# sksundaram-learning/linkerd

Measured on AMD Instinct MI355X. Metric: histogram samples ingested+summarized/sec (1M series) and % HBM peak, higher is better.
Workload: dtype u32; 1 GPU; C3: 1M series, 1e9 Zipf(s=1) samples per step, log-normal values; series_total=1000000, series_per_gpu=1000000, rotating_batches=3, parallelism=series-sharded x1 (weighted ranges), step=ingest (sample+plan+bin1+bin2) + snapshot(reset, dense counts + summaries)

## Files before the change

linkerd_amd/csrc/l5dh_engine.cpp:

```cpp
#include <algorithm>
#include <cerrno>
#include <cstring>
#include <mutex>
#include <new>
#include <string>
#include <vector>

#include "l5dh_ctx.hpp"

using namespace l5dh;

namespace {

constexpr size_t MAX_BATCH = ((size_t)1 << 30) - 65536;

hipEvent_t ev_get(l5dh_ctx* c) {
  if (!c->ev_pool.empty()) {
    hipEvent_t e = c->ev_pool.back();
    c->ev_pool.pop_back();
    return e;
  }
  hipEvent_t e = nullptr;
  hipEventCreate(&e);
  return e;
// ... 113 lines not shown
  Segs sv = segs_view(c);
  size_t recs = 0;
  for (int j = 0; j < c->nseg; ++j) recs += c->segs[j].n;
  uint32_t hc = c->hot_chunk;
  {
    const size_t fill = recs / (2 * (size_t)std::max(1, c->num_cu));
    hc = (uint32_t)std::min<size_t>(hc, std::max<size_t>(16384, (fill + 1023) & ~(size_t)1023));
  }
  if (int r = ensure(c, c->split_item, (recs / hc + 2 * (size_t)c->F + 2) * 8)) return r;
  Plan pl = plan(c);
  const int direct_out = final_mode && reset && out.counts && out.first == 0 && out.count == (uint32_t)c->S;
  if (encode && !(final_mode && reset && out.first == 0 && out.count == (uint32_t)c->S && !out.counts && !out.summ))
    return fail(c, -EINVAL, "internal: the sparse export is a whole-range resetting export");
  {
    KTimer kt(c, L5DH_K_SCAN);
    if (encode) HIPCHK(c, launch_enc_dirty(state(c), pl, c->stream));
    HIPCHK(c, launch_plan(sv, c->F, final_mode, c->cold_limit, hc, c->d_dirty, direct_out, encode ? 1 : 0, pl,
                          c->stream));
  }
  if (encode) {
    uint32_t words = 0;
    HIPCHK(c, hipMemcpyAsync(&words, c->d_header + 5 + 4 * ((c->F + 1023) / 1024), 4, hipMemcpyDeviceToHost,
                             c->stream));
    HIPCHK(c, hipStreamSynchronize(c->stream));
    if (int r = ensure(c, c->m_unpacked, (size_t)words * 4 + 16)) return r;
    c->m_unpacked_words = words;
    out.enc = c->m_unpacked.as<uint32_t>();
  }
  const uint32_t hot = (uint32_t)std::min<size_t>(c->F, recs / ((size_t)c->cold_limit + 1));
  const uint32_t split_items = (uint32_t)std::min<size_t>(0xFFFFFFF0u, recs / hc + 2 * (size_t)hot);
  State st = state(c);
  Tables tb = tables(c);
  if (hot) {
    KTimer kt(c, L5DH_K_HOT);
    HIPCHK(c, launch_hot_init(pl, hot, st, out, direct_out, c->stream));
  }
  bool joined = true;
  {
    KTimer kt(c, L5DH_K_ACCUM);
    const bool big_seen = __atomic_load_n(c->h_header + 5, __ATOMIC_RELAXED) != 0u;
    if (split_items && big_seen) {
      HIPCHK(c, hipEventRecord(c->ev_fork, c->stream));
      HIPCHK(c, hipStreamWaitEvent(c->side, c->ev_fork, 0));
      HIPCHK(c, launch_accum_split(sv, pl, split_items, st, tb, out, direct_out, hc, c->stream));
      HIPCHK(c, launch_accum_cold(sv, pl, DEV_COUNT, st, tb, out, final_mode, reset, c->side));
      HIPCHK(c, hipEventRecord(c->ev_join, c->side));
      joined = false;
    } else {
      if (split_items) HIPCHK(c, launch_accum_split(sv, pl, split_items, st, tb, out, direct_out, hc, c->stream));
      HIPCHK(c, launch_accum_cold(sv, pl, DEV_COUNT, st, tb, out, final_mode, reset, c->stream));
    }
    if (hot) HIPCHK(c, launch_hot_finish(pl, hot, st, tb, out, final_mode, reset, direct_out, c->stream));
    if (!joined) HIPCHK(c, hipStreamWaitEvent(c->stream, c->ev_join, 0));
  }
  c->nseg = 0;
  return 0;
}

int flush_ring(l5dh_ctx* c) {
  if (!c->ring_fill) return 0;
  const size_t n = c->ring_fill;
  c->ring_fill = 0;
  return do_ingest(c, c->ring_series.as<const uint32_t>(), c->ring_values.as<const float>(), n);
}

}

namespace {

int fold(l5dh_ctx* c) {
  Outputs none{nullptr, nullptr, 0, 0, nullptr};
  return aggregate(c, 0, 0, none);
}

int check_err(l5dh_ctx* c) {
  const uint32_t seen = __atomic_load_n(c->h_header + 4, __ATOMIC_ACQUIRE);
  if (seen != c->err_reported) {
    c->err_reported = seen;
    return fail(c, -EINVAL, "series id >= max_series in an ingest batch (those samples were dropped)");
  }
  return 0;
}

int do_ingest(l5dh_ctx* c, const uint32_t* series, const float* values, size_t n) {
  if (n == 0) return 0;
  if (n > MAX_BATCH) return fail(c, -EINVAL, "batch piece larger than 2^30 samples");
  if (c->nseg >= c->max_seg) {
    int r = fold(c);
    if (r) return r;
  }
  const uint32_t* ds = series;
  const float* dv = values;
  if (!is_device_ptr(series) || !is_device_ptr(values)) {
    int r;
    if ((r = ensure(c, c->stage_series, n * 4))) return r;
    if ((r = ensure(c, c->stage_values, n * 4))) return r;
    KTimer kt(c, L5DH_K_COPY);
    HIPCHK(c, hipMemcpyAsync(c->stage_series.p, series, n * 4, hipMemcpyDefault, c->stream));
    HIPCHK(c, hipMemcpyAsync(c->stage_values.p, values, n * 4, hipMemcpyDefault, c->stream));
    ds = c->stage_series.as<const uint32_t>();
    dv = c->stage_values.as<const float>();
  }
  const bool vec = ((uintptr_t)ds % 16 == 0) && ((uintptr_t)dv % 16 == 0);
  if (c->F == 1) {
    KTimer kt(c, L5DH_K_BIN);
    const size_t fill = n / (size_t)std::max(1, c->num_cu);
    const uint32_t chunk =
        (uint32_t)std::min<size_t>(c->hot_chunk & ~3u, std::max<size_t>(16384, (fill + 1023) & ~(size_t)1023));
    HIPCHK(c, launch_fold1(ds, dv, n, chunk, state(c), tables(c), c->d_err, vec, (c->variant & 1) != 0, c->stream));
    c->fold_last = n;
    HIPCHK(c, hipMemcpyAsync(c->h_header + 4, c->d_err, 4, hipMemcpyDeviceToHost, c->stream));
    return 0;
  }
  auto& sg = c->segs[c->nseg];
  const size_t cap32 = n + n / 2 + ((size_t)1 << 19);
  const size_t cap16 = 2 * n + n / 8 + (size_t)128 * c->F + 4096;
  const size_t dlim16 = (cap16 - (n + (size_t)16 * c->F + 1024)) & ~(size_t)7;
  {
    int r = ensure(c, sg.rec32, (cap32 + 16) * 4);
    if (!r) r = ensure(c, sg.rec16, (cap16 + 16) * 2);
    if (r) return r;
  }
  int G = (int)std::min<size_t>((size_t)c->G_max, (n + 8191) / 8192);
  if (G < 1) G = 1;
  size_t per = (n + G - 1) / G;
  per = (per + 3) & ~(size_t)3;
  G = (int)((n + per - 1) / per);
  IngestArgs a{};
  a.series = ds;
  a.values = dv;
  a.n = n;
  a.per = per;
  a.G = G;
  a.num_cu = c->num_cu;
  a.S = c->S;
  a.F = c->F;
  a.tb = tables(c);
  a.sumfix = c->d_sumfix;
  a.err = c->d_err;
  a.err_host = c->h_header_dev + 4;
  a.kest = c->d_kest;
  a.kprev = c->d_kprev;
  a.meta = sg.meta;
  a.rec32 = sg.rec32.as<uint32_t>();
  a.rec16 = sg.rec16.as<uint16_t>();
  a.cap32 = cap32;
  a.cap16 = cap16;
  a.dlim16 = dlim16;
  a.thr_min = (uint32_t)std::min<uint64_t>(std::max<uint64_t>(1, n / (8192ull * c->direct_div)), 0xFFFFFFFFull);
  const uint32_t FS = (c->F + 63) / 64;
  a.dmax = std::min<uint32_t>(c->direct_max, ((uint32_t)BIN1_BINS - 9 - FS) / 2);
  a.pct = c->region_pct;
  a.vec = vec;
  {
    KTimer kt(c, L5DH_K_SCAN);
    if (c->variant & 4) HIPCHK(c, hipMemsetAsync(c->d_kprev, 0, (size_t)2 * c->F * 4, c->stream));
    HIPCHK(c, launch_ingest(a, 0, c->stream));
  }
  {
    KTimer kt(c, L5DH_K_BIN);
    HIPCHK(c, launch_ingest(a, 1, c->stream));
  }
  {
    KTimer kt(c, L5DH_K_BIN2);
    HIPCHK(c, launch_ingest(a, 3, c->stream));
  }
  sg.n = n;
  c->nseg++;
  return 0;
}

int wait_inputs(l5dh_ctx* c) {
  HIPCHK(c, hipEventRecord(c->ev_copy, c->stream));
  HIPCHK(c, hipEventSynchronize(c->ev_copy));
  return 0;
}

int issue_ticket(l5dh_ctx* c, uint64_t* ticket) {
  const uint64_t t = ++c->tick_next;
  const int slot = (int)(t % l5dh_ctx::NTICK);
  if (!c->tick_ev[slot]) HIPCHK(c, hipEventCreateWithFlags(&c->tick_ev[slot], hipEventDisableTiming));
  HIPCHK(c, hipEventRecord(c->tick_ev[slot], c->stream));
  c->tick_of[slot] = t;
  *ticket = t;
  return 0;
}

int wait_ticket(l5dh_ctx* c, uint64_t t) {
  if (t <= c->tick_done) return 0;
  if (t > c->tick_next) return fail(c, -EINVAL, "unknown ingest ticket");
  const int slot = (int)(t % l5dh_ctx::NTICK);
  HIPCHK(c, hipEventSynchronize(c->tick_ev[slot]));
  c->tick_done = std::max(c->tick_done, c->tick_of[slot]);
  return 0;
}

int ingest_impl(l5dh_ctx* c, const uint32_t* series, const float* values, size_t n, uint64_t* ticket = nullptr) {
  if (ticket) *ticket = c->tick_next;
  if (n == 0) return 0;
  const bool dev = is_device_ptr(series) && is_device_ptr(values);
  const bool wait = (!dev || c->stream == c->own_stream) && !ticket;
  if (c->ring_cap && n <= c->ring_cap / 2) {
    int r;
    if (c->ring_fill + n > c->ring_cap && (r = flush_ring(c))) return r;
    if ((r = ensure(c, c->ring_series, c->ring_cap * 4 + 64)) || (r = ensure(c, c->ring_values, c->ring_cap * 4 + 64)))
      return r;
    {
      KTimer kt(c, L5DH_K_COPY);
      uint32_t* rs = c->ring_series.as<uint32_t>() + c->ring_fill;
      float* rv = c->ring_values.as<float>() + c->ring_fill;
      const void* hs = dev || (c->variant & 2) ? nullptr : host_mapped_ptr(series);
      const void* hv = hs ? host_mapped_ptr(values) : nullptr;
      if (hs && hv) {
        HIPCHK(c, launch_fetch_host(static_cast<const uint32_t*>(hs), static_cast<const uint32_t*>(hv), rs,
                                    reinterpret_cast<uint32_t*>(rv), n, c->stream));
      } else {
        HIPCHK(c, hipMemcpyAsync(rs, series, n * 4, hipMemcpyDefault, c->stream));
        HIPCHK(c, hipMemcpyAsync(rv, values, n * 4, hipMemcpyDefault, c->stream));
      }
    }
    c->ring_fill += n;
    if (ticket) return issue_ticket(c, ticket);
    return wait ? wait_inputs(c) : 0;
  }
  int r = flush_ring(c);
  if (r) return r;
  for (size_t o = 0; o < n; o += MAX_BATCH) {
    const size_t m = std::min(n - o, MAX_BATCH);
    if ((r = do_ingest(c, series + o, values + o, m))) return r;
  }
  if (ticket) return issue_ticket(c, ticket);
  return wait ? wait_inputs(c) : 0;
}

bool full_range(l5dh_ctx* c, uint32_t first, uint32_t count) { return first == 0 && count == c->S; }

int do_snapshot(l5dh_ctx* c, uint32_t first, uint32_t count, l5dh_summary* out, int32_t* counts_out, int reset) {
  if ((uint64_t)first + count > c->S) return fail(c, -EINVAL, "series range out of bounds");
  if (count == 0) return 0;
  int r = flush_ring(c);
  if (r) return r;
  StagedOut<Summary88> summ;
  StagedOut<int32_t> cnt;
  if ((r = summ.begin(c, out, count, c->stage_summ)) || (r = cnt.begin(c, counts_out, (size_t)count * NB, c->stage_counts)))
    return r;
  Outputs o{summ.dev, cnt.dev, first, count, nullptr};
  if (full_range(c, first, count) && c->F > 1) {
    if ((r = aggregate(c, 1, reset, o))) return r;
  } else {
    if ((r = fold(c))) return r;
    KTimer kt(c, L5DH_K_HOT);
    HIPCHK(c, launch_rows(state(c), nullptr, nullptr, tables(c), o, reset, nullptr, c->stream));
  }
  {
    KTimer kt(c, L5DH_K_COPY);
    if ((r = summ.end(c)) || (r = cnt.end(c))) return r;
  }
  if (!summ.staged() && !cnt.staged() && c->stream != c->own_stream) return 0;
  return sync_stream(c);
}

int do_rollup(l5dh_ctx* c, uint32_t first, uint32_t count, const int32_t* ext, const int64_t* ext_totals,
              const uint32_t* group, uint32_t G, l5dh_summary* g_out, int32_t* g_counts_out, int64_t* g_totals_out,
              l5dh_summary* series_out, int reset) {
  int r;
  const bool live = ext == nullptr;
  if (live && ((r = flush_ring(c)) || (r = fold(c)))) return r;
  RollupWork w{};
  w.count = count;
  w.G = G;
  w.first = first;
  w.item = c->rollup_item;
  w.caps = rollup_caps(count, G, w.item);
  w.tmp_bytes = rollup_tmp_bytes(G);
  const size_t G1 = (size_t)G + 1;
  if ((r = ensure(c, c->ru_u32, (4 * G1 + RH_WORDS) * 4)) || (r = ensure(c, c->ru_u64, 2 * G1 * 8)) ||
      (r = ensure(c, c->ru_members, ((size_t)count + 1) * 4)) || (r = ensure(c, c->ru_igroup, w.caps.items * 4)) ||
      (r = ensure(c, c->ru_mlist, (w.caps.multi + 1) * 4)) ||
      (r = ensure(c, c->ru_partial, (w.caps.slots + 1) * (size_t)RU_PROW * 8)) ||
      (r = ensure(c, c->ru_tmp, w.tmp_bytes)))
    return r;
  {
    KTimer kt(c, L5DH_K_COPY);
    if ((r = stage_in(c, group, count, 4, c->ru_group)) ||
        (r = stage_in(c, ext, (size_t)count * NB, 8, c->stage_in_counts)) ||
        (r = stage_in(c, ext_totals, count, 8, c->stage_in_totals)))
      return r;
  }
  w.group = group;
  uint32_t* u = c->ru_u32.as<uint32_t>();
  w.cnt = u;
  w.nitems = u + G1;
  w.cursor = u + 2 * G1;
  w.pbase = u + 3 * G1;
  w.hdr = u + 4 * G1;
  w.moff = c->ru_u64.as<uint64_t>();
  w.ioff = w.moff + G1;
  w.members = c->ru_members.as<uint32_t>();
  w.igroup = c->ru_igroup.as<uint32_t>();
  w.mlist = c->ru_mlist.as<uint32_t>();
  w.partial = c->ru_partial.as<uint64_t>();
  w.tmp = c->ru_tmp.p;
  StagedOut<Summary88> g_summ, s_summ;
  StagedOut<int32_t> g_cnt;
  StagedOut<int64_t> g_tot;
  if ((r = g_summ.begin(c, g_out, G, c->ru_summ)) || (r = g_cnt.begin(c, g_counts_out, (size_t)G * NB, c->ru_counts)) ||
// ... 507 lines not shown
```

linkerd_amd/csrc/l5dh_ingest.hip:

```cpp
#include <algorithm>
#include <type_traits>

#include "l5dh_device.hpp"

namespace l5dh {
namespace {

constexpr uint32_t RSAMPLE = 1u << 18;
#ifndef L5DH_RS_WG
#define L5DH_RS_WG 64
#endif
constexpr int RS_WG = L5DH_RS_WG;
static_assert((RSAMPLE + RS_WG - 1) / RS_WG <= 65535, "k_rsample's u16 LDS counters: at most 65535 draws per workgroup");
constexpr uint32_t INVALID = 0xFFFFFFFFu;

__device__ __forceinline__ uint32_t round_up(uint32_t x, uint32_t m) { return (x + m - 1) / m * m; }

__device__ __forceinline__ uint32_t rcap(double prev, double e, double s, bool exact, double pad, uint32_t align,
                                         uint32_t pct, double z, bool floor_sample) {
  double c;
  if (exact) {
    c = e;
  } else {
    const double e0 = prev / s, sg = sqrt(e0 + 1.0);
// ... 112 lines not shown
      } else if (t < F) {
        x[i].x = kw[2 * t];
        x[i].y = kw[2 * t + 1];
      }
    }
  };
  uint2 te[16];
  {
    uint4 x[16];
    load_pairs(kest, x);
#pragma unroll
    for (int i = 0; i < 16; ++i) te[i] = make_uint2(x[i].x + x[i].y, x[i].z + x[i].w);
  }
  auto scaled = [&](uint32_t v) -> uint32_t { return (uint32_t)fmin((double)v * s, 4294967295.0); };
  __syncthreads();
  RP_MARK(1)
  auto hist = [&](uint32_t v) {
    const uint32_t e = scaled(v);
    const bool ok = dmax > 0 && e >= thr_min && e > 0;
    const int bin = ok ? 31 - __clz((int)e) : 0;
    const uint64_t act = __ballot(ok);
    if (!act) return;
    const int b0 = __builtin_amdgcn_readlane(bin, __builtin_ctzll(act));
    if (__ballot(ok && bin == b0) == act) {
      if (lane == 0) atomicAdd(&lh[b0], (uint32_t)__popcll(act));
    } else if (ok) {
      atomicAdd(&lh[bin], 1u);
    }
  };
#pragma unroll
  for (int i = 0; i < 16; ++i) {
    hist(te[i].x);
    hist(te[i].y);
  }
  __syncthreads();
  if (j < 64) {
    const uint32_t c = j < 32 ? lh[31 - j] : 0u;
    const uint32_t cum = wave_incl_scan32(c);
    const uint64_t ok = __ballot(dmax > 0 && j < 32 && cum <= dmax);
    const int nb = __popcll(ok);
    if (j == 0) sthr = nb ? max(max(thr_min, 1u), 1u << (32 - nb)) : 0xFFFFFFFFu;
  }
#pragma unroll
  for (int i = 0; i < 16; ++i) reinterpret_cast<uint2*>(tw)[j + 1024u * (uint32_t)i] = te[i];
  uint4 xp[16];
  load_pairs(kprev, xp);
  __syncthreads();
  const uint32_t thr = sthr;
  RP_MARK(2)
  uint32_t dbits = 0, E = 0;
#pragma unroll
  for (int k = 0; k < 32; ++k) {
    const uint32_t kk = (uint32_t)(k + (int)j) & 31u;
    const uint32_t v = tw[t0 + kk];
    if (t0 + kk < F && scaled(v) >= thr) dbits |= 1u << kk;
    else E += v;
  }
  __syncthreads();
#pragma unroll
  for (int i = 0; i < 16; ++i)
    reinterpret_cast<uint2*>(tw)[j + 1024u * (uint32_t)i] = make_uint2(xp[i].x + xp[i].y, xp[i].z + xp[i].w);
  __syncthreads();
  uint64_t P = 0;
#pragma unroll
  for (int k = 0; k < 32; ++k) {
    const uint32_t kk = (uint32_t)(k + (int)j) & 31u;
    if (!((dbits >> kk) & 1u)) P += tw[t0 + kk];
  }
  RP_MARK(3)
  uint32_t cv[4] = {(uint32_t)__popc(dbits), 0u, 0u, 0u}, ct[4];
  block_excl_scan4<1024>(cv, lds4, ct);
  const uint32_t ND = ct[0];
  meta[L.dbits() + j] = j < NW ? dbits : 0u;
  meta[L.dpre() + j] = cv[0];
  {
    uint32_t x = dbits, di = cv[0];
    while (x) {
      const uint32_t k = (uint32_t)(__ffs((int)x) - 1);
      x &= x - 1u;
      dl[di] = t0 + k;
      meta[L.dlist() + di] = t0 + k;
      ++di;
    }
  }
  P += __shfl_xor(P, 1, 64);
  E += __shfl_xor(E, 1, 64);
  RP_MARK(4)
  if ((j & 1u) == 0 && (j >> 1) < FS) {
    const uint32_t b = j >> 1;
    capl[b] = rcap((double)P, (double)E, s, exact, 256.0, 4, pct, 6.0, true);
    meta[L.btot() + b] = (uint32_t)min(P, (uint64_t)0xFFFFFFFFu);
  }
  __syncthreads();
  RP_MARK(5)
  const uint32_t TB = FS + 2 * ND;
  if (j >= FS && j < TB) {
    const uint32_t t = dl[(j - FS) >> 1], h = (j - FS) & 1u;
    const double p = (double)kprev[2 * t + h], e = (double)kest[2 * t + h];
    capl[j] = rcap(p, e, s, exact, 256.0, 8, pct, 5.0, false);
  }
  __syncthreads();
  const bool stb = j < FS, dj = j >= FS && j < TB;
  uint64_t tot32, tot16;
  const uint64_t base32 = block_excl_scan64(stb ? (uint64_t)capl[j] : 0ull, l64, &tot32);
  const uint64_t base16 = block_excl_scan64(dj ? (uint64_t)capl[j] : 0ull, l64, &tot16);
  const uint64_t base = stb ? base32 : base16;
  const uint64_t lim = stb ? cap32 : dlim16;
  if (base + capl[j] + 16 > lim)
    capl[j] = base + 16 < lim ? (uint32_t)(lim - 16 - base) & (stb ? ~3u : ~7u) : 0u;
  meta[L.bbase() + j] = (uint32_t)base;
  meta[L.bcap() + j] = j < TB ? capl[j] : 0u;
  meta[L.bcnt() + j] = 0u;
  if (j == 0) {
    uint32_t* hdr = meta + L.hdr();
    hdr[H_ND] = ND;
    hdr[H_OV1] = 0;
    hdr[H_REDO1] = 0;
    hdr[H_OV2] = 0;
    hdr[H_REDO2] = 0;
    hdr[H_COUNT2] = 0;
    hdr[H_EXACT] = exact ? 1u : 0u;
    hdr[H_D16] = (uint32_t)min(tot16, (uint64_t)dlim16);
  }
  RP_MARK(6)
}




#ifdef L5DH_PHASES
__device__ unsigned long long g_phase1[1024 * 8];
__device__ unsigned long long g_phase3[1024 * 8];
#define PH_INIT unsigned long long ph_acc[7] = {0, 0, 0, 0, 0, 0, 0}, ph_t = wall_clock64();
#define PH_VWAIT asm volatile("s_waitcnt vmcnt(0)" ::: "memory");
#define PH_MARK(k)                                 \
  if (threadIdx.x == 0) {                          \
    const unsigned long long ph_n = wall_clock64(); \
    ph_acc[k] += ph_n - ph_t;                      \
    ph_t = ph_n;                                   \
  }
#define PH_FLUSH                                                                   \
  if (threadIdx.x == 0 && pass == 0) {                                             \
    for (int k = 0; k < 7; ++k) g_phase1[blockIdx.x * 8 + k] += ph_acc[k];          \
    g_phase1[blockIdx.x * 8 + 7] += 1;                                             \
  }
#else
#define PH_INIT
#define PH_MARK(k)
#define PH_VWAIT
#define PH_FLUSH
#endif
__device__ __forceinline__ uint4 ld_stream(const uint32_t* p) { return *reinterpret_cast<const uint4*>(p); }
constexpr int CHW = 16384;
using dsum_t = unsigned long long;
constexpr uint32_t NODEST = 0xFFFFFFFFu - (uint32_t)CHW;
constexpr int NT1 = 1024;
constexpr int DSUM_N = DIRECT_MAX * TILE;
constexpr size_t rbin1w_lds() {
  return (size_t)CHW * 4 + BIN1_BINS * 12 + CHW / 8 + CHW / 32 + 1024 * 8 + LUT2_N * 8 + DSUM_N * sizeof(dsum_t);
}

template <int NT, int CH>
__global__ __launch_bounds__(NT) void k_rbin1w(const uint32_t* __restrict__ series, const float* __restrict__ values,
                                                  size_t n, size_t per, uint32_t S, uint32_t F, Tables tb,
                                                  uint32_t* __restrict__ meta, uint32_t* __restrict__ rec32,
                                                  uint16_t* __restrict__ rec16, int64_t* __restrict__ sumfix,
                                                  uint32_t* __restrict__ err, int vec, int pass) {
  constexpr int PT = CH / NT;
  constexpr int PH = PT / 2;
  constexpr int GS = 4;
  static_assert(PH % 4 == 0 && PH % GS == 0 && GS % 4 == 0 && CH <= 32768, "halves of whole 16-B groups; 15-bit ranks");
  extern __shared__ __attribute__((aligned(16))) uint32_t smem[];
  uint32_t* stage = smem;
  uint32_t* cnt = stage + CH;
  uint32_t* offr = cnt + BIN1_BINS;
  uint32_t* rdelta = offr + BIN1_BINS;
  uint32_t* heads = rdelta + BIN1_BINS;
  uint16_t* gpre = reinterpret_cast<uint16_t*>(heads + CH / 32);
  uint2* dw = reinterpret_cast<uint2*>(gpre + CH / 64);
  uint2* lut2 = dw + 1024;
  __shared__ uint32_t wsum[NT / 64];
  dsum_t* dsum = reinterpret_cast<dsum_t*>(lut2 + LUT2_N);
  const MetaLayout L = meta_layout(F);
  uint32_t* hdr = meta + L.hdr();
  if (pass == 1 && __builtin_amdgcn_readfirstlane(hdr[H_REDO1]) == 0u) return;
  uint32_t* bcnt = meta + L.bcnt();
  const uint32_t* bbase = meta + L.bbase();
  const uint32_t* bcap = meta + L.bcap();
  const uint32_t FS = (F + ST_TILES - 1) / ST_TILES;
  const uint32_t NW = (F + 31) / 32;
  const uint32_t ND = hdr[H_ND];
  const uint32_t TB = FS + 2 * ND;
  const int lane = lane_id();
  const int wv = threadIdx.x >> 6;
  for (uint32_t w = threadIdx.x; w < NW; w += NT) dw[w] = make_uint2(meta[L.dbits() + w], meta[L.dpre() + w]);
  for (uint32_t b = threadIdx.x; b < BIN1_BINS; b += NT) cnt[b] = 0;
  for (uint32_t i = threadIdx.x; i < LUT2_N; i += NT) lut2[i] = tb.lut2[i];
  for (uint32_t i = threadIdx.x; i < ND * TILE; i += NT) dsum[i] = 0;
  __syncthreads();
  const uint32_t lo = (uint32_t)((size_t)blockIdx.x * per);
  const uint32_t hi = (uint32_t)min((size_t)lo + per, n);
  bool bad = false;
  constexpr int RB0 = (BIN1_BINS + NT - 1) / NT;
  uint32_t my_base[RB0], my_cap[RB0];
#pragma unroll
  for (int j = 0; j < RB0; ++j) {
    const uint32_t b = threadIdx.x + (uint32_t)j * NT;
    my_base[j] = b < TB ? bbase[b] : 0u;
    my_cap[j] = b < TB ? bcap[b] : 0u;
  }
  PH_INIT
  constexpr int PFG = PH / 4;
  uint4 pfs[PFG], pfv[PFG];
  auto prefetch = [&](uint32_t c) {
#pragma unroll
    for (int k = 0; k < PFG; ++k) {
      const uint32_t base = c + 4u * ((uint32_t)k * NT + threadIdx.x);
      pfs[k] = ld_stream(series + base);
      pfv[k] = ld_stream(reinterpret_cast<const uint32_t*>(values) + base);
    }
  };
  if (vec && lo + (uint32_t)CH <= hi) prefetch(lo);
  for (uint32_t c0 = lo; c0 < hi; c0 += CH) {
    for (uint32_t wd = threadIdx.x; wd < CH / 32; wd += NT) heads[wd] = 0u;
    uint32_t pk[PT];
    const bool full = vec && c0 + (uint32_t)CH <= hi;
    const uint32_t cl = c0;
    uint4 hs[PH / 4], hv[PH / 4];
    auto load_second = [&]() {
      if (full) {
#pragma unroll
        for (int k = 0; k < PH / 4; ++k) {
          const uint32_t base = cl + 4u * ((uint32_t)(PH / 4 + k) * NT + threadIdx.x);
          hs[k] = ld_stream(series + base);
          hv[k] = ld_stream(reinterpret_cast<const uint32_t*>(values) + base);
        }
      }
    };
#pragma unroll
    for (int h = 0; h < 2; ++h) {
      if (h == 1) { PH_MARK(1) }
      uint32_t sv[PH];
      float fv[PH];
      if (full) {
#pragma unroll
        for (int k = 0; k < PH / 4; ++k) {
          uint4 s4, u4;
          if (h == 0) {
            s4 = pfs[h * (PH / 4) + k];
            u4 = pfv[h * (PH / 4) + k];
          } else {
            s4 = hs[k];
            u4 = hv[k];
          }
          const float4 f4 = make_float4(__uint_as_float(u4.x), __uint_as_float(u4.y), __uint_as_float(u4.z),
                                        __uint_as_float(u4.w));
          sv[4 * k] = s4.x; sv[4 * k + 1] = s4.y; sv[4 * k + 2] = s4.z; sv[4 * k + 3] = s4.w;
          fv[4 * k] = f4.x; fv[4 * k + 1] = f4.y; fv[4 * k + 2] = f4.z; fv[4 * k + 3] = f4.w;
        }
      } else {
#pragma unroll
        for (int k = 0; k < PH; ++k) {
          const uint32_t i = c0 + 4u * ((uint32_t)(h * (PH / 4) + (k >> 2)) * NT + threadIdx.x) + (uint32_t)(k & 3);
          const bool in = i < hi;
          sv[k] = in ? series[i] : 0xFFFFFFFFu;
          fv[k] = in ? values[i] : 0.0f;
          bad |= in && sv[k] >= S;
        }
      }
      if (full) {
        PH_VWAIT
        if (h == 0) { PH_MARK(0) } else { PH_MARK(2) }
      }
#pragma unroll
      for (int g = 0; g < PH; g += GS) {
        if (h == 0 && g == GS) load_second();
        uint32_t pl[GS];
        uint32_t escm = 0;
#pragma unroll
        for (int q = 0; q < GS; ++q) {
          const float f = fv[g + q];
          const bool fast = __float_as_uint(f) < 0x49FFC000u;
          pl[q] = fast ? (uint32_t)f : 0u;
          escm |= (!fast && sv[g + q] < S) ? (1u << q) : 0u;
          if (full) bad |= sv[g + q] >= S;
        }
        if (__ballot(escm != 0u)) {
#pragma unroll 1
          for (int q = 0; q < GS; ++q) {
            if ((escm >> q) & 1u) {
              const uint32_t i = cl + 4u * ((uint32_t)(h * (PH / 4) + (g + q) / 4) * NT + threadIdx.x) + (uint32_t)(q & 3);
              const uint32_t r = payload1_slow(series[i], values[i], tb, pass == 0 ? sumfix : nullptr);
#pragma unroll
              for (int u = 0; u < GS; ++u) pl[u] = q == u ? r : pl[u];
            }
          }
        }
        uint2 dv[GS], lv[GS];
#pragma unroll
        for (int q = 0; q < GS; ++q) dv[q] = dw[(sv[g + q] >> (TILE_SHIFT + 5)) & 1023u];
#pragma unroll
        for (int q = 0; q < GS; ++q) lv[q] = lut2[lut2_index(pl[q])];
        uint32_t rc4[GS];
#pragma unroll
        for (int q = 0; q < GS; ++q) {
          const uint32_t s = sv[g + q];
          const uint32_t tw = __builtin_amdgcn_ubfe(s, TILE_SHIFT, 5);
          const bool direct = s < S && __builtin_amdgcn_ubfe(dv[q].x, tw, 1) != 0u;
          const uint32_t di = dv[q].y + (uint32_t)__popc(__builtin_amdgcn_ubfe(dv[q].x, 0, tw));
          const uint32_t p = pl[q];
          uint32_t o;
          const uint32_t bk = lut2_decode(p, lv[q], o);
          const bool esc = p >= V_ESC;
          const uint32_t bucket = sel_u32(esc, p - V_ESC, bk);
          rc4[q] = sel_u32(direct, ((s & (TILE - 1)) << 11) | bucket, ((s & (ST_TILES * TILE - 1)) << 21) | p);
          const uint32_t dbin = FS + 2u * di + ((s >> 4) & 1u);
          const uint32_t bn = sel_u32(s < S, sel_u32(direct, dbin, s >> ST_SHIFT), TB);
          pk[h * PH + g + q] = atomicAdd(cnt + bn, 1u) | (bn << 15);
          if (direct && !esc && pass == 0 && p) atomicAdd(&dsum[di * TILE + (s & (TILE - 1))], (dsum_t)p);
        }
#pragma unroll
        for (int j = 0; j < GS / 4; ++j)
          *reinterpret_cast<uint4*>(stage + 4u * ((uint32_t)(h * (PH / 4) + g / 4 + j) * NT + threadIdx.x)) =
              make_uint4(rc4[4 * j], rc4[4 * j + 1], rc4[4 * j + 2], rc4[4 * j + 3]);
        asm volatile("" ::: "memory");
      }
    }
    __syncthreads();
    PH_MARK(3)
    constexpr int RB = (BIN1_BINS + NT - 1) / NT;
    uint32_t rn[RB], rold[RB], rbase[RB], rcapv[RB];
#pragma unroll
    for (int j = 0; j < RB; ++j) {
      const uint32_t rb_bin = threadIdx.x + (uint32_t)j * NT;
      rn[j] = rb_bin <= TB ? cnt[rb_bin] : 0u;
      rold[j] = 0;
      rbase[j] = my_base[j];
      rcapv[j] = my_cap[j];
      if (rb_bin < TB && rn[j]) rold[j] = atomicAdd(&bcnt[rb_bin], rn[j]);
    }
    {
      static_assert(NT == BIN1_BINS && RB == 1, "one bin per thread");
      const uint32_t pv = rn[0] | ((rn[0] ? 1u : 0u) << 16);
      const uint32_t wi = wave_incl_scan32(pv);
      if (lane == 63) wsum[wv] = wi;
      __syncthreads();
      uint32_t pre = 0;
      for (int q = 0; q < wv; ++q) pre += wsum[q];
      const uint32_t ex = pre + wi - pv;
      offr[threadIdx.x] = ex;
      if (rn[0]) atomicOr(&heads[(ex & 0xFFFFu) >> 5], 1u << (ex & 31u));
    }
    uint32_t rec[PT];
#pragma unroll
    for (int kk = 0; kk < PT / 4; ++kk) {
      const uint4 v = *reinterpret_cast<const uint4*>(stage + 4u * ((uint32_t)kk * NT + threadIdx.x));
      rec[4 * kk] = v.x; rec[4 * kk + 1] = v.y; rec[4 * kk + 2] = v.z; rec[4 * kk + 3] = v.w;
    }
    __syncthreads();
    PH_MARK(4)
    if (vec && c0 + 2u * (uint32_t)CH <= hi) prefetch(c0 + (uint32_t)CH);
#pragma unroll
    for (int k = 0; k < PT; ++k) {
      const uint32_t bin = (pk[k] >> 15) & 1023u;
      stage[(offr[bin] & 0xFFFFu) + (pk[k] & 0x7FFFu)] = rec[k];
    }
    if (wv == 0) {
      constexpr int GPL = CH / 64 / 64;
      static_assert(GPL % 2 == 0, "two groups per 16-B read");
      uint32_t pc[GPL], t = 0;
#pragma unroll
      for (int k = 0; k < GPL; k += 2) {
        const uint4 w = *reinterpret_cast<const uint4*>(heads + 2u * (GPL * (uint32_t)lane + (uint32_t)k));
        pc[k] = (uint32_t)(__popc(w.x) + __popc(w.y));
        pc[k + 1] = (uint32_t)(__popc(w.z) + __popc(w.w));
        t += pc[k] + pc[k + 1];
      }
      uint32_t ex = wave_incl_scan32(t) - t;
#pragma unroll
      for (int k = 0; k < GPL; ++k) {
        gpre[GPL * (uint32_t)lane + (uint32_t)k] = (uint16_t)ex;
        ex += pc[k];
      }
    }
#pragma unroll
    for (int j = 0; j < RB; ++j) {
      const uint32_t rb_bin = threadIdx.x + (uint32_t)j * NT;
      if (rn[j]) {
        uint32_t d = NODEST;
        if (rb_bin < TB) {
          if (rold[j] + rn[j] <= rcapv[j]) d = rbase[j] + rold[j] - (offr[rb_bin] & 0xFFFFu);
          else hdr[H_OV1] = 1u;
        }
        rdelta[offr[rb_bin] >> 16] = d;
      }
    }
    __syncthreads();
    PH_MARK(5)
    const uint32_t nst = offr[FS] >> 16;
#pragma unroll
    for (int j = 0; j < RB; ++j)
      if (threadIdx.x + (uint32_t)j * NT < BIN1_BINS) cnt[threadIdx.x + (uint32_t)j * NT] = 0;
#pragma unroll 4
    for (int k = 0; k < PT; ++k) {
      const uint32_t i = (uint32_t)wv * (PT * 64) + (uint32_t)k * 64 + (uint32_t)lane;
      const uint32_t g = i >> 6;
      const unsigned long long hw = *reinterpret_cast<const unsigned long long*>(heads + 2 * g);
      const uint32_t run = (uint32_t)gpre[g] + mask_below(hw) + (uint32_t)((hw >> lane) & 1ull) - 1u;
      const uint32_t d = rdelta[run];
      if (d != NODEST) {
        if (run < nst)
          rec32[i + d] = stage[i];
        else
          rec16[i + d] = (uint16_t)stage[i];
      }
    }
    __syncthreads();
    PH_MARK(6)
  }
  PH_FLUSH
  if (pass == 0) {
    const uint32_t* dl = meta + L.dlist();
    for (uint32_t i = threadIdx.x; i < ND * TILE; i += NT) {
      const unsigned long long v = dsum[i];
      const uint32_t s = dl[i / TILE] * TILE + (i & (TILE - 1));
      if (v && s < S) atomicAdd(reinterpret_cast<unsigned long long*>(&sumfix[s]), (unsigned long long)v);
    }
    if (bad) atomicAdd(err, 1u);
  }
}

__device__ __forceinline__ uint32_t lut3_byte(uint32_t v) {
  const uint32_t sh = 25u - (uint32_t)__builtin_clz(v | 64u);
  return ((v >> sh) + (sh << 6)) << 3;
}
__device__ __forceinline__ uint32_t lut3_bucket(uint32_t v, uint2 x) {
  return (x.x & 0x7FFu) + (((v << 11) | 0x7FFu) >= x.x ? 1u : 0u) + (v >= x.y ? 1u : 0u);
}

__global__ __launch_bounds__(1024) void k_rfix1(uint32_t F, uint32_t* __restrict__ meta, const uint32_t* __restrict__ err,
                                                uint32_t* __restrict__ err_host) {
  __shared__ uint32_t lds[17];
  const MetaLayout L = meta_layout(F);
  uint32_t* hdr = meta + L.hdr();
  if (threadIdx.x == 0) *reinterpret_cast<volatile uint32_t*>(err_host) = *err;
  const uint32_t FS = (F + ST_TILES - 1) / ST_TILES;
  const uint32_t ND = hdr[H_ND];
  const uint32_t TB = FS + 2 * ND;
  const uint32_t ov = hdr[H_OV1];
  const uint32_t b = threadIdx.x;
  const bool stb = b < FS, dj = b >= FS && b < TB;
  const uint32_t c = b < TB ? meta[L.bcnt() + b] : 0u;
  if (stb && !hdr[H_EXACT]) {
    const double P = (double)meta[L.btot() + b];
    if ((double)c > P * 1.0625 + 4.0 * sqrt(P) + 256.0) hdr[H_COUNT2] = 1u;
  }
  meta[L.btot() + b] = c;
  uint32_t t32, t16;
  const uint32_t nb32 = block_excl_scan<1024>(stb ? round_up(c, 4) : 0u, lds, &t32);
  const uint32_t nb16 = block_excl_scan<1024>(dj ? round_up(c, 8) : 0u, lds, &t16);
  const uint32_t nb = stb ? nb32 : nb16;
  const uint32_t base = ov ? nb : meta[L.bbase() + b];
  if (dj) {
    const uint32_t t = meta[L.dlist() + ((b - FS) >> 1)], h = (b - FS) & 1u;
    meta[L.kbase() + 2 * t + h] = base;
    meta[L.kcnt() + 2 * t + h] = c;
  }
  if (ov) {
    meta[L.bbase() + b] = nb;
    meta[L.bcap() + b] = round_up(c, stb ? 4 : 8);
    meta[L.bcnt() + b] = 0u;
  }
  const uint32_t d16 = hdr[H_D16];
  if (ov && t16 > d16) {
    for (uint32_t k = b; k < L.K; k += 1024)
      if (!((meta[L.dbits() + (k >> 6)] >> ((k >> 1) & 31u)) & 1u)) meta[L.kcap() + k] = 0u;
  }
  uint32_t all;
  const uint32_t is = block_excl_scan<1024>(stb ? (c + ITEM2 - 1) / ITEM2 : 0u, lds, &all);
  if (stb) meta[L.istart() + b] = is;
  __syncthreads();
  if (b == 0) {
    meta[L.istart() + FS] = all;
    hdr[H_ITEMS] = all;
    if (ov && t16 > d16) {
      hdr[H_D16] = t16;
      hdr[H_COUNT2] = 1u;
    }
    hdr[H_OV2] = 0u;
    hdr[H_REDO2] = 0u;
    hdr[H_REDO1] = ov;
    hdr[H_OV1] = 0u;
    if (ov) hdr[H_NOVR1] += 1u;
  }
}

__device__ __forceinline__ bool tile_direct(const uint32_t* __restrict__ meta, const MetaLayout& L, uint32_t t) {
  return (meta[L.dbits() + (t >> 5)] >> (t & 31u)) & 1u;
// ... 301 lines not shown
    if (wv < 2) {
      uint32_t rb = INVALID;
      if (rc) {
        if (rold + rc <= rcapv) rb = rbase + rold;
        else hdr[H_OV2] = 1u;
      }
      ocx[b * B2_KEYS + rk].y = rb;
      cnt[rk] = 0u;
    }
    __syncthreads();
    PH2_MARK(4)
    prev_total = ctot;
#pragma unroll
    for (int g = 0; g < PG; ++g) x[g] = xn[g];
  }
  write_out((int)((i1 - 1) & 1u), prev_total);
  __syncthreads();
  if (pass == 0) flush(cur_j);
#ifdef L5DH_PHASES
  if (threadIdx.x == 0 && pass == 0) {
    for (int k = 0; k < 5; ++k) g_phase3[blockIdx.x * 8 + k] += ph2[k];
    g_phase3[blockIdx.x * 8 + 7] += 1;
  }
#endif
}

__global__ __launch_bounds__(1024) void k_rfix2a(uint32_t F, uint32_t* __restrict__ meta, uint32_t* __restrict__ kprev) {
  __shared__ uint64_t red[16];
  const MetaLayout L = meta_layout(F);
  uint32_t* hdr = meta + L.hdr();
  const uint32_t k = blockIdx.x * 1024u + threadIdx.x;
  uint32_t r8 = 0;
  if (k < L.K) {
    const uint32_t c = meta[L.kcnt() + k];
    kprev[k] = c;
    if (!tile_direct(meta, L, k >> 1)) r8 = round_up(c, 8);
  }
  const uint64_t w = wave_sum((uint64_t)r8);
  if ((threadIdx.x & 63) == 0) red[threadIdx.x >> 6] = w;
  __syncthreads();
  if (threadIdx.x == 0) {
    uint64_t t = 0;
    for (int q = 0; q < 16; ++q) t += red[q];
    reinterpret_cast<uint64_t*>(meta + L.wsum())[blockIdx.x] = t;
    if (blockIdx.x == 0) hdr[H_REDO2] = hdr[H_OV2] | hdr[H_COUNT2];
  }
}

__global__ __launch_bounds__(1024) void k_rfix2b(uint32_t F, uint32_t* __restrict__ meta) {
  __shared__ uint64_t red[16];
  __shared__ uint64_t l64[17];
  const MetaLayout L = meta_layout(F);
  uint32_t* hdr = meta + L.hdr();
  if (hdr[H_REDO2] == 0u) return;
  const uint64_t before = wsum_before(reinterpret_cast<const uint64_t*>(meta + L.wsum()), blockIdx.x, red);
  const uint32_t k = blockIdx.x * 1024u + threadIdx.x;
  const bool mine = k < L.K && !tile_direct(meta, L, k >> 1);
  const uint32_t c8 = mine ? round_up(meta[L.kcnt() + k], 8) : 0u;
  uint64_t total;
  const uint64_t base = hdr[H_D16] + before + block_excl_scan64((uint64_t)c8, l64, &total);
  if (mine) {
    meta[L.kbase() + k] = (uint32_t)base;
    meta[L.kcap() + k] = c8;
    meta[L.kcnt() + k] = 0u;
  }
  if (blockIdx.x == 0 && threadIdx.x == 0) {
    if (hdr[H_COUNT2]) hdr[H_NCNT2] += 1u;
    else hdr[H_NOVR2] += 1u;
    hdr[H_OV2] = 0u;
  }
}

__global__ __launch_bounds__(1024) void k_rfix2s(uint32_t F, uint32_t* __restrict__ meta, uint32_t* __restrict__ kprev) {
  __shared__ uint64_t l64[17];
  const MetaLayout L = meta_layout(F);
  uint32_t* hdr = meta + L.hdr();
  constexpr uint32_t KPM = RFIX2_ONE_WG_MAX / 1024;
  const uint32_t KP = (L.K + 1023) / 1024, k0 = threadIdx.x * KP;
  const uint32_t redo = hdr[H_OV2] | hdr[H_COUNT2];
  const uint32_t counted = hdr[H_COUNT2];
  uint32_t c8[KPM], dm = 0;
  uint64_t mine = 0;
#pragma unroll
  for (uint32_t q = 0; q < KPM; ++q) {
    const uint32_t k = k0 + q;
    c8[q] = 0;
    if (q < KP && k < L.K) {
      const uint32_t c = meta[L.kcnt() + k];
      kprev[k] = c;
      if (tile_direct(meta, L, k >> 1)) {
        dm |= 1u << q;
      } else {
        c8[q] = round_up(c, 8);
        mine += c8[q];
      }
    }
  }
  __syncthreads();
  if (threadIdx.x == 0) hdr[H_REDO2] = redo;
  if (!redo) return;
  uint64_t total;
  uint64_t kb = (uint64_t)hdr[H_D16] + block_excl_scan64(mine, l64, &total);
#pragma unroll
  for (uint32_t q = 0; q < KPM; ++q) {
    const uint32_t k = k0 + q;
    if (q < KP && k < L.K && !((dm >> q) & 1u)) {
      meta[L.kbase() + k] = (uint32_t)kb;
      meta[L.kcap() + k] = c8[q];
      meta[L.kcnt() + k] = 0u;
      kb += c8[q];
    }
  }
  if (threadIdx.x == 0) {
    if (counted) hdr[H_NCNT2] += 1u;
    else hdr[H_NOVR2] += 1u;
    hdr[H_OV2] = 0u;
  }
}

__global__ __launch_bounds__(256) void k_fetch_host(const uint32_t* __restrict__ hs, const uint32_t* __restrict__ hv,
                                                    uint32_t* __restrict__ ds, uint32_t* __restrict__ dv, size_t n) {
  const size_t stride = (size_t)gridDim.x * blockDim.x;
  for (size_t i = (size_t)blockIdx.x * blockDim.x + threadIdx.x; i < n; i += stride) {
    const uint32_t s = hs[i], v = hv[i];
    ds[i] = s;
    dv[i] = v;
  }
}

}

#ifdef L5DH_PHASES
extern "C" __attribute__((visibility("default"))) int l5dh_dev_phases3(unsigned long long* out) {
  return (int)hipMemcpyFromSymbol(out, HIP_SYMBOL(g_phase3), sizeof(g_phase3), 0, hipMemcpyDeviceToHost);
}
extern "C" __attribute__((visibility("default"))) int l5dh_dev_phases_plan(unsigned long long* out) {
  return (int)hipMemcpyFromSymbol(out, HIP_SYMBOL(g_phase_plan), sizeof(g_phase_plan), 0, hipMemcpyDeviceToHost);
}
extern "C" __attribute__((visibility("default"))) int l5dh_dev_phases1(unsigned long long* out) {
  return (int)hipMemcpyFromSymbol(out, HIP_SYMBOL(g_phase1), sizeof(g_phase1), 0, hipMemcpyDeviceToHost);
}
#endif

hipError_t launch_fetch_host(const uint32_t* hs, const uint32_t* hv, uint32_t* ds, uint32_t* dv, size_t n,
                             hipStream_t st) {
  if (n == 0) return hipSuccess;
  const size_t blocks = std::min<size_t>((n + 255) / 256, 2048);
  hipLaunchKernelGGL(k_fetch_host, dim3((unsigned)blocks), dim3(256), 0, st, hs, hv, ds, dv, n);
  return hipGetLastError();
}

hipError_t set_ingest_attributes() {
  hipError_t e;
  if ((e = hipFuncSetAttribute((const void*)k_rsample, hipFuncAttributeMaxDynamicSharedMemorySize, 32768 * 4)))
    return e;
  if ((e = hipFuncSetAttribute((const void*)k_rplan1, hipFuncAttributeMaxDynamicSharedMemorySize, (int)RPLAN1_LDS)))
    return e;
  return hipFuncSetAttribute((const void*)k_rbin1w<NT1, CHW>, hipFuncAttributeMaxDynamicSharedMemorySize,
                             (int)rbin1w_lds());
}

hipError_t launch_ingest(const IngestArgs& a, int stage, hipStream_t st) {
  const uint32_t K = 2 * a.F;
  switch (stage) {
    case 0:
      hipLaunchKernelGGL(k_rsample, dim3(RS_WG), dim3(1024), (size_t)((K + 1) / 2) * 4, st, a.series, a.n, a.S, K,
                         a.kest);
      hipLaunchKernelGGL(k_rplan1, dim3(1), dim3(1024), RPLAN1_LDS, st, a.n, a.F, a.kest, a.kprev, a.meta, a.cap32,
                         a.dlim16, a.thr_min, a.dmax, a.pct);
      {
        const uint32_t B = (K + 1023) / 1024;
        hipLaunchKernelGGL(k_rplan2a, dim3(B), dim3(1024), 0, st, a.n, a.F, a.kest, a.kprev, a.meta, a.pct);
        hipLaunchKernelGGL(k_rplan2b, dim3(B), dim3(1024), 0, st, a.F, a.meta, a.cap16);
      }
      break;
    case 1:
      for (int pass = 0; pass < 2; ++pass) {
        hipLaunchKernelGGL((k_rbin1w<NT1, CHW>), dim3(a.G), dim3(NT1), rbin1w_lds(), st, a.series, a.values, a.n,
                           a.per, a.S, a.F, a.tb, a.meta, a.rec32, a.rec16, a.sumfix, a.err, a.vec ? 1 : 0, pass);
        if (pass == 0) hipLaunchKernelGGL(k_rfix1, dim3(1), dim3(1024), 0, st, a.F, a.meta, a.err, a.err_host);
      }
      break;
    case 2:
      break;
    default: {
      const uint32_t B = (K + 1023) / 1024;
      for (int pass = 0; pass < 2; ++pass) {
        const MetaLayout L = meta_layout(a.F);
        hipLaunchKernelGGL(k_rbin2<B2_NT>, dim3(a.num_cu * B2_PER_CU), dim3(B2_NT), 0, st, a.S, a.F, a.tb, a.meta,
                           a.meta + L.istart(), a.meta + L.bbase(), a.meta + L.btot(), a.rec32, a.rec16, a.sumfix,
                           pass);
        if (pass == 0 && K <= RFIX2_ONE_WG_MAX) {
          hipLaunchKernelGGL(k_rfix2s, dim3(1), dim3(1024), 0, st, a.F, a.meta, a.kprev);
        } else if (pass == 0) {
          hipLaunchKernelGGL(k_rfix2a, dim3(B), dim3(1024), 0, st, a.F, a.meta, a.kprev);
          hipLaunchKernelGGL(k_rfix2b, dim3(B), dim3(1024), 0, st, a.F, a.meta);
        }
      }
      break;
    }
  }
  return hipGetLastError();
}

}
```

linkerd_amd/csrc/l5dh_kernels.hpp:

```cpp
#pragma once

#include <hip/hip_runtime.h>

#include <cstddef>
#include <cstdint>

#include "l5dh_tables.hpp"

namespace l5dh {

constexpr int TILE = 32;
constexpr int TILE_SHIFT = 5;
constexpr int ST_TILES = 64;
constexpr int ST_SHIFT = 11;
constexpr int CROW = 900;
constexpr int HROW = 1800;
constexpr int MAX_SEG = 8;
constexpr int WG = 1024;
constexpr uint32_t COLD_LIMIT_MAX = 65535u;

constexpr size_t ACC_COLDH_LDS = (size_t)16 * CROW * 4 + 16 * 8 + ROW * 4;
constexpr int ENC_LIST = 256;
constexpr size_t ACC_COLDHE_LDS = ACC_COLDH_LDS + 2 * 16 * 4 + (size_t)16 * ENC_LIST * 2;
constexpr size_t ACC_SPLIT_LDS = (size_t)16 * HROW * 4;
constexpr size_t FOLD16_LDS = (size_t)16 * HROW * 4 + 16 * 64 * 8 + 1024 * 8;
constexpr size_t FOLD32_LDS = (size_t)TILE * CROW * 4 + TILE * 64 * 8 + 1024 * 8;

struct Tables {
  const int32_t* lim_pad;
  const int32_t* mid;
  const int32_t* base;
  const uint32_t* lut;
  const uint2* lut2;
  const uint2* lut3;
};

constexpr int DIRECT_MAX = 255;
constexpr int BIN1_BINS = 1024;
constexpr uint32_t ITEM2 = 6144;
struct MetaLayout {
  uint32_t K;
  __host__ __device__ constexpr uint32_t kbase() const { return 0; }
  __host__ __device__ constexpr uint32_t kcnt() const { return K; }
  __host__ __device__ constexpr uint32_t kcap() const { return 2 * K; }
  __host__ __device__ constexpr uint32_t dbits() const { return 3 * K; }
  __host__ __device__ constexpr uint32_t dpre() const { return 3 * K + 1024; }
  __host__ __device__ constexpr uint32_t dlist() const { return 3 * K + 2048; }
  __host__ __device__ constexpr uint32_t bbase() const { return 3 * K + 2304; }
  __host__ __device__ constexpr uint32_t bcnt() const { return 3 * K + 3328; }
  __host__ __device__ constexpr uint32_t bcap() const { return 3 * K + 4352; }
  __host__ __device__ constexpr uint32_t btot() const { return 3 * K + 5376; }
  __host__ __device__ constexpr uint32_t hdr() const { return 3 * K + 6400; }
  __host__ __device__ constexpr uint32_t istart() const { return 3 * K + 6464; }
  __host__ __device__ constexpr uint32_t wsum() const { return 3 * K + 6980; }
  __host__ __device__ constexpr uint32_t words() const { return 3 * K + 7108; }
};
__host__ __device__ constexpr MetaLayout meta_layout(uint32_t F) { return MetaLayout{2 * F}; }
enum : uint32_t {
  H_ND = 0,
  H_OV1 = 1,
  H_REDO1 = 2,
  H_OV2 = 3,
  H_REDO2 = 4,
  H_ITEMS = 5,
  H_COUNT2 = 6,
  H_EXACT = 9,
  H_NOVR1 = 10,
  H_NOVR2 = 11,
  H_D16 = 12,
  H_NCNT2 = 13
};
constexpr uint32_t NOKEY = 0xFFFFFFFFu;

struct Segs {
  const uint16_t* rec16[MAX_SEG];
  const uint32_t* meta[MAX_SEG];
  int n;
};

struct Summary88 {
  int64_t count, min, max, sum, p50, p90, p95, p99, p9990, p9999;
  double avg;
};
static_assert(sizeof(Summary88) == 88, "HistogramSummary layout");

struct State {
  uint32_t* counts;
  int64_t* total;
  int64_t* sumfix;
  uint8_t* dirty;
  uint32_t S, F;
};

constexpr uint32_t CI_DIRTY = 1u << 30;
constexpr uint8_t TF_SPLIT = 2;
constexpr uint8_t TF_DIRTY = 4;
constexpr uint8_t TF_SOLO = 8;

struct Plan {
  uint32_t* tile_tot;
  uint32_t* enc_base;
  uint32_t* enc_h0;
  uint32_t* enc_dw;
  uint4* cold_item;
  uint2* split_item;
  uint32_t* hot_list;
  uint8_t* tile_flags;
  uint32_t* header;
  uint32_t* big_hint;
};
__host__ __device__ constexpr uint32_t plan_header_words(uint32_t F) { return 6 + 4 * ((F + 1023) / 1024); }
constexpr uint32_t ENC_HALF_CAP = 16u * 2u * NB + 16u;
static_assert((uint64_t)((1u << 20) / TILE) * 2u * ENC_HALF_CAP < (1ull << 32),
              "the unpacked encoding's u32 word offsets (L5DH_MAX_SERIES = 2^20 series)");

struct Outputs {
  Summary88* summ;
  int32_t* counts;
  uint32_t first, count;
  int64_t* totals;
  uint32_t* words;
  uint32_t* enc;
  uint32_t* roff;
};
constexpr uint32_t MERGE_CMAX = 0x1FFFFFu;

struct IngestArgs {
  const uint32_t* series;
  const float* values;
  size_t n, per;
  int G;
  int num_cu;
  uint32_t S, F;
  Tables tb;
  int64_t* sumfix;
  uint32_t* err;
  uint32_t* err_host;
  uint32_t* kest;
  uint32_t* kprev;
  uint32_t* meta;
  uint32_t* rec32;
  uint16_t* rec16;
  size_t cap32, cap16;
  size_t dlim16;
  uint32_t thr_min, dmax;
  uint32_t pct;
  bool vec;
};
hipError_t launch_ingest(const IngestArgs& a, int stage, hipStream_t st);
hipError_t set_ingest_attributes();

hipError_t launch_fold1(const uint32_t* series, const float* values, size_t n, uint32_t chunk, State state, Tables tb,
                        uint32_t* err, bool vec, bool wide, hipStream_t st);

hipError_t launch_enc_dirty(State st, Plan plan, hipStream_t st_);
hipError_t launch_plan(Segs segs, uint32_t F, int final_mode, uint32_t cold_limit, uint32_t hot_chunk,
                       const uint8_t* dirty, int direct_out, int encode, Plan plan, hipStream_t st);
constexpr uint32_t DEV_COUNT = 0xFFFFFFFFu;
hipError_t launch_hot_init(Plan plan, uint32_t max_hot, State state, Outputs out, int direct_out, hipStream_t st);
hipError_t launch_accum_cold(Segs segs, Plan plan, uint32_t cold_items, State state, Tables tb, Outputs out,
                             int final_mode, int reset, hipStream_t st);
hipError_t launch_accum_split(Segs segs, Plan plan, uint32_t max_split_items, State state, Tables tb,
                              Outputs out, int direct_out, uint32_t hot_chunk, hipStream_t st);
hipError_t launch_hot_finish(Plan plan, uint32_t max_hot, State state, Tables tb, Outputs out, int final_mode,
                             int reset, int direct_out, hipStream_t st);
hipError_t launch_rows(State state, const int32_t* ext, const int64_t* ext_total, Tables tb, Outputs out,
                       int reset, int64_t* totals_out, hipStream_t st);
hipError_t launch_fetch_host(const uint32_t* hs, const uint32_t* hv, uint32_t* ds, uint32_t* dv, size_t n,
                             hipStream_t st);
hipError_t set_snapshot_attributes();

}
```

Measured before the change: 174.5 billion samples/s.

## Use u32 LDS direct-sum accumulators with overflow-triggered flushes in bin1

Templates the bin1 kernel on the direct-sum accumulator type and makes u32 the default, with the old u64 path kept behind a variant bit. Halving the width of the LDS atomics and storage is meant to cut LDS atomic cost. Overflow is bounded by lowering the fast-path float threshold, so larger payloads go straight to global sumfix atomics. Each direct bin also tracks per-bin arrival counts and flushes its partial sums to global sumfix once the count exceeds the chunk size. This adds extra LDS state, extra flush logic, and more global atomics for mid-sized values.

```diff
diff --git a/linkerd_amd/csrc/l5dh_engine.cpp b/linkerd_amd/csrc/l5dh_engine.cpp
--- a/linkerd_amd/csrc/l5dh_engine.cpp
+++ b/linkerd_amd/csrc/l5dh_engine.cpp
@@ -289,6 +289,7 @@
   a.dmax = std::min<uint32_t>(c->direct_max, ((uint32_t)BIN1_BINS - 9 - FS) / 2);
   a.pct = c->region_pct;
   a.vec = vec;
+  a.dsum64 = (c->variant & 8) != 0;
   {
     KTimer kt(c, L5DH_K_SCAN);
     if (c->variant & 4) HIPCHK(c, hipMemsetAsync(c->d_kprev, 0, (size_t)2 * c->F * 4, c->stream));
diff --git a/linkerd_amd/csrc/l5dh_ingest.hip b/linkerd_amd/csrc/l5dh_ingest.hip
--- a/linkerd_amd/csrc/l5dh_ingest.hip
+++ b/linkerd_amd/csrc/l5dh_ingest.hip
@@ -288,15 +288,18 @@
 #endif
 __device__ __forceinline__ uint4 ld_stream(const uint32_t* p) { return *reinterpret_cast<const uint4*>(p); }
 constexpr int CHW = 16384;
-using dsum_t = unsigned long long;
+constexpr uint32_t DSUM_PMAX = 1u << 17;
+static_assert(DSUM_PMAX == 1u << 17, "the ranking loop tests the bits of 2^17f, 0x48000000");
 constexpr uint32_t NODEST = 0xFFFFFFFFu - (uint32_t)CHW;
 constexpr int NT1 = 1024;
 constexpr int DSUM_N = DIRECT_MAX * TILE;
-constexpr size_t rbin1w_lds() {
-  return (size_t)CHW * 4 + BIN1_BINS * 12 + CHW / 8 + CHW / 32 + 1024 * 8 + LUT2_N * 8 + DSUM_N * sizeof(dsum_t);
-}
-
-template <int NT, int CH>
+constexpr size_t rbin1w_lds(size_t dsz) {
+  return (size_t)CHW * 4 + BIN1_BINS * 12 + CHW / 8 + CHW / 32 + 1024 * 8 + LUT2_N * 8 + DSUM_N * dsz +
+         (dsz == 4 ? (size_t)BIN1_BINS * 12 : 0);
+}
+static_assert(rbin1w_lds(4) <= 160 * 1024 && rbin1w_lds(8) <= 160 * 1024, "one workgroup's LDS");
+
+template <int NT, int CH, typename DS>
 __global__ __launch_bounds__(NT) void k_rbin1w(const uint32_t* __restrict__ series, const float* __restrict__ values,
                                                   size_t n, size_t per, uint32_t S, uint32_t F, Tables tb,
                                                   uint32_t* __restrict__ meta, uint32_t* __restrict__ rec32,
@@ -306,6 +309,9 @@
   constexpr int PH = PT / 2;
   constexpr int GS = 4;
   static_assert(PH % 4 == 0 && PH % GS == 0 && GS % 4 == 0 && CH <= 32768, "halves of whole 16-B groups; 15-bit ranks");
+  constexpr bool S32 = sizeof(DS) == 4;
+  static_assert(!S32 || (2ull * CH * (DSUM_PMAX - 1) < (1ull << 32) && CH <= CHW),
+                "u32 direct sums: <= CH (2^17 - 1) at a sub-chunk's start + as much from the sub-chunk");
   extern __shared__ __attribute__((aligned(16))) uint32_t smem[];
   uint32_t* stage = smem;
   uint32_t* cnt = stage + CH;
@@ -316,7 +322,9 @@
   uint2* dw = reinterpret_cast<uint2*>(gpre + CH / 64);
   uint2* lut2 = dw + 1024;
   __shared__ uint32_t wsum[NT / 64];
-  dsum_t* dsum = reinterpret_cast<dsum_t*>(lut2 + LUT2_N);
+  DS* dsum = reinterpret_cast<DS*>(lut2 + LUT2_N);
+  uint32_t* dacc = reinterpret_cast<uint32_t*>(dsum + DSUM_N);
+  uint2* breg = reinterpret_cast<uint2*>(dacc + BIN1_BINS);
   const MetaLayout L = meta_layout(F);
   uint32_t* hdr = meta + L.hdr();
   if (pass == 1 && __builtin_amdgcn_readfirstlane(hdr[H_REDO1]) == 0u) return;
@@ -330,7 +338,10 @@
   const int lane = lane_id();
   const int wv = threadIdx.x >> 6;
   for (uint32_t w = threadIdx.x; w < NW; w += NT) dw[w] = make_uint2(meta[L.dbits() + w], meta[L.dpre() + w]);
-  for (uint32_t b = threadIdx.x; b < BIN1_BINS; b += NT) cnt[b] = 0;
+  for (uint32_t b = threadIdx.x; b < BIN1_BINS; b += NT) {
+    cnt[b] = 0;
+    if (S32) dacc[b] = 0;
+  }
   for (uint32_t i = threadIdx.x; i < LUT2_N; i += NT) lut2[i] = tb.lut2[i];
   for (uint32_t i = threadIdx.x; i < ND * TILE; i += NT) dsum[i] = 0;
   __syncthreads();
@@ -344,6 +355,7 @@
     const uint32_t b = threadIdx.x + (uint32_t)j * NT;
     my_base[j] = b < TB ? bbase[b] : 0u;
     my_cap[j] = b < TB ? bcap[b] : 0u;
+    if (S32) breg[b] = make_uint2(my_base[j], my_cap[j]);
   }
   PH_INIT
   constexpr int PFG = PH / 4;
@@ -416,7 +428,7 @@
 #pragma unroll
         for (int q = 0; q < GS; ++q) {
           const float f = fv[g + q];
-          const bool fast = __float_as_uint(f) < 0x49FFC000u;
+          const bool fast = __float_as_uint(f) < (S32 ? 0x48000000u : 0x49FFC000u);
           pl[q] = fast ? (uint32_t)f : 0u;
           escm |= (!fast && sv[g + q] < S) ? (1u << q) : 0u;
           if (full) bad |= sv[g + q] >= S;
@@ -426,7 +438,13 @@
           for (int q = 0; q < GS; ++q) {
             if ((escm >> q) & 1u) {
               const uint32_t i = cl + 4u * ((uint32_t)(h * (PH / 4) + (g + q) / 4) * NT + threadIdx.x) + (uint32_t)(q & 3);
-              const uint32_t r = payload1_slow(series[i], values[i], tb, pass == 0 ? sumfix : nullptr);
+              const uint32_t si = series[i];
+              const uint32_t r = payload1_slow(si, values[i], tb, pass == 0 ? sumfix : nullptr);
+              if (S32 && pass == 0 && r - DSUM_PMAX < V_ESC - DSUM_PMAX) {
+                const uint2 d = dw[(si >> (TILE_SHIFT + 5)) & 1023u];
+                if ((d.x >> ((si >> TILE_SHIFT) & 31u)) & 1u)
+                  atomicAdd(reinterpret_cast<unsigned long long*>(&sumfix[si]), (unsigned long long)r);
+              }
 #pragma unroll
               for (int u = 0; u < GS; ++u) pl[u] = q == u ? r : pl[u];
             }
@@ -453,7 +471,11 @@
           const uint32_t dbin = FS + 2u * di + ((s >> 4) & 1u);
           const uint32_t bn = sel_u32(s < S, sel_u32(direct, dbin, s >> ST_SHIFT), TB);
           pk[h * PH + g + q] = atomicAdd(cnt + bn, 1u) | (bn << 15);
-          if (direct && !esc && pass == 0 && p) atomicAdd(&dsum[di * TILE + (s & (TILE - 1))], (dsum_t)p);
+          if (S32) {
+            if (direct && pass == 0 && p - 1u < DSUM_PMAX - 1u) atomicAdd(&dsum[di * TILE + (s & (TILE - 1))], (DS)p);
+          } else if (direct && !esc && pass == 0 && p) {
+            atomicAdd(&dsum[di * TILE + (s & (TILE - 1))], (DS)p);
+          }
         }
 #pragma unroll
         for (int j = 0; j < GS / 4; ++j)
@@ -466,20 +488,46 @@
     PH_MARK(3)
     constexpr int RB = (BIN1_BINS + NT - 1) / NT;
     uint32_t rn[RB], rold[RB], rbase[RB], rcapv[RB];
+    uint32_t tq = threadIdx.x;
+    if (S32) asm volatile("" : "+v"(tq));
 #pragma unroll
     for (int j = 0; j < RB; ++j) {
-      const uint32_t rb_bin = threadIdx.x + (uint32_t)j * NT;
+      const uint32_t rb_bin = tq + (uint32_t)j * NT;
       rn[j] = rb_bin <= TB ? cnt[rb_bin] : 0u;
       rold[j] = 0;
-      rbase[j] = my_base[j];
-      rcapv[j] = my_cap[j];
+      if (S32) {
+        const uint2 r = breg[rb_bin];
+        rbase[j] = r.x;
+        rcapv[j] = r.y;
+      } else {
+        rbase[j] = my_base[j];
+        rcapv[j] = my_cap[j];
+      }
       if (rb_bin < TB && rn[j]) rold[j] = atomicAdd(&bcnt[rb_bin], rn[j]);
+    }
+    if (S32 && pass == 0) {
+      bool fl = false;
+      if (tq >= FS && tq < TB && rn[0]) {
+        const uint32_t A = dacc[tq] + rn[0];
+        fl = A > (uint32_t)CH;
+        dacc[tq] = fl ? 0u : A;
+      }
+      for (uint64_t fm = __ballot(fl); fm; fm &= fm - 1) {
+        const uint32_t fb = (tq & ~63u) + (uint32_t)__builtin_ctzll(fm) - FS;
+        if ((tq & 63u) < TILE / 2) {
+          const uint32_t h = fb * (TILE / 2) + (tq & 63u);
+          const uint32_t v = (uint32_t)dsum[h];
+          dsum[h] = 0;
+          const uint32_t sr = meta[L.dlist() + h / TILE] * TILE + (h & (TILE - 1));
+          if (v && sr < S) atomicAdd(reinterpret_cast<unsigned long long*>(&sumfix[sr]), (unsigned long long)v);
+        }
+      }
     }
     {
       static_assert(NT == BIN1_BINS && RB == 1, "one bin per thread");
       const uint32_t pv = rn[0] | ((rn[0] ? 1u : 0u) << 16);
       const uint32_t wi = wave_incl_scan32(pv);
-      if (lane == 63) wsum[wv] = wi;
+      if ((tq & 63u) == 63u) wsum[tq >> 6] = wi;
       __syncthreads();
       uint32_t pre = 0;
       for (int q = 0; q < wv; ++q) pre += wsum[q];
@@ -1087,12 +1135,15 @@
 
 hipError_t set_ingest_attributes() {
   hipError_t e;
+  if ((e = hipFuncSetAttribute((const void*)k_rbin1w<NT1, CHW, unsigned long long>,
+                               hipFuncAttributeMaxDynamicSharedMemorySize, (int)rbin1w_lds(8))))
+    return e;
   if ((e = hipFuncSetAttribute((const void*)k_rsample, hipFuncAttributeMaxDynamicSharedMemorySize, 32768 * 4)))
     return e;
   if ((e = hipFuncSetAttribute((const void*)k_rplan1, hipFuncAttributeMaxDynamicSharedMemorySize, (int)RPLAN1_LDS)))
     return e;
-  return hipFuncSetAttribute((const void*)k_rbin1w<NT1, CHW>, hipFuncAttributeMaxDynamicSharedMemorySize,
-                             (int)rbin1w_lds());
+  return hipFuncSetAttribute((const void*)k_rbin1w<NT1, CHW, uint32_t>, hipFuncAttributeMaxDynamicSharedMemorySize,
+                             (int)rbin1w_lds(4));
 }
 
 hipError_t launch_ingest(const IngestArgs& a, int stage, hipStream_t st) {
@@ -1111,8 +1162,14 @@
       break;
     case 1:
       for (int pass = 0; pass < 2; ++pass) {
-        hipLaunchKernelGGL((k_rbin1w<NT1, CHW>), dim3(a.G), dim3(NT1), rbin1w_lds(), st, a.series, a.values, a.n,
-                           a.per, a.S, a.F, a.tb, a.meta, a.rec32, a.rec16, a.sumfix, a.err, a.vec ? 1 : 0, pass);
+        if (a.dsum64)
+          hipLaunchKernelGGL((k_rbin1w<NT1, CHW, unsigned long long>), dim3(a.G), dim3(NT1), rbin1w_lds(8), st, a.series,
+                             a.values, a.n, a.per, a.S, a.F, a.tb, a.meta, a.rec32, a.rec16, a.sumfix, a.err,
+                             a.vec ? 1 : 0, pass);
+        else
+          hipLaunchKernelGGL((k_rbin1w<NT1, CHW, uint32_t>), dim3(a.G), dim3(NT1), rbin1w_lds(4), st, a.series,
+                             a.values, a.n, a.per, a.S, a.F, a.tb, a.meta, a.rec32, a.rec16, a.sumfix, a.err,
+                             a.vec ? 1 : 0, pass);
         if (pass == 0) hipLaunchKernelGGL(k_rfix1, dim3(1), dim3(1024), 0, st, a.F, a.meta, a.err, a.err_host);
       }
       break;
diff --git a/linkerd_amd/csrc/l5dh_kernels.hpp b/linkerd_amd/csrc/l5dh_kernels.hpp
--- a/linkerd_amd/csrc/l5dh_kernels.hpp
+++ b/linkerd_amd/csrc/l5dh_kernels.hpp
@@ -146,6 +146,7 @@
   uint32_t thr_min, dmax;
   uint32_t pct;
   bool vec;
+  bool dsum64;
 };
 hipError_t launch_ingest(const IngestArgs& a, int stage, hipStream_t st);
 hipError_t set_ingest_attributes();
```

New measurement: 178.1 billion samples/s (median of 6 runs). +2.1%, better.
